# Vandermode/TFPnP

Measured on AMD Instinct MI355X. Metric: PnP-ADMM iters/sec (and images/sec) at env_batch=48, 256x256, 30 inner iters, higher is better.
Workload: dtype f32 (v_mfma_f32_32x32x2_f32; Winograd F(2x2,3x3) on the layers with cout % 32 == 0); 1 GPU; CS-MRI ADMM 256x256 env_batch=48/GPU radial x4 sigma_n=15, 6 solver calls x 5 inner iters + PSNR reward, no early stop; global_batch=48, parallelism=single GPU

## Files before the change

### include/pnpx.h

```cpp
#ifndef PNPX_H
#define PNPX_H

#include <stddef.h>
#include <stdint.h>

#ifdef __cplusplus
extern "C" {
#endif

typedef struct pnpx_ctx pnpx_ctx;

enum pnpx_status {
  PNPX_OK = 0,
  PNPX_ERR_ARG = 1,
  PNPX_ERR_SHAPE = 2,
  PNPX_ERR_NO_WEIGHTS = 3,
  PNPX_ERR_ALLOC = 4,
  PNPX_ERR_HIP = 5,
  PNPX_ERR_RANGE = 6
};

const char* pnpx_version(void);
const char* pnpx_last_error(void);

// ... 167 lines not shown
int pnpx_spi_admm_train(pnpx_ctx* ctx, const float* vars_in, float* vars_out, const float* x0, const float* Kmap,
                        const float* sigma_d, const float* mu, int param_stride, int B, int H, int W, int T,
                        float* saved, unsigned long long* ticket, void* stream);
int pnpx_spi_admm_backward(pnpx_ctx* ctx, const float* x0, const float* Kmap, const float* sigma_d, const float* mu,
                           int param_stride, const float* saved, const float* grad_vars_out, float* grad_vars_in,
                           float* grad_sigma_d, float* grad_mu, float* work, int B, int H, int W, int T,
                           unsigned long long ticket, void* stream);

int pnpx_radon_det_count(int R);
int pnpx_radon_forward(pnpx_ctx* ctx, const float* img, float* sino, int B, int R, int n_view, void* stream);
int pnpx_radon_backprojection(pnpx_ctx* ctx, const float* sino, float* img, int B, int R, int n_view,
                              void* stream);
int pnpx_ct_iadmm(pnpx_ctx* ctx, const float* vars_in, float* vars_out, const float* y0, int n_view,
                  float opnorm, const float* sigma_d, const float* mu, const float* tau, int param_stride,
                  int B, int R, int T, void* stream);
int pnpx_ct_iadmm_train(pnpx_ctx* ctx, const float* vars_in, float* vars_out, const float* y0, int n_view,
                        float opnorm, const float* sigma_d, const float* mu, const float* tau, int param_stride, int B,
                        int R, int T, float* saved, unsigned long long* ticket, void* stream);
int pnpx_ct_iadmm_backward(pnpx_ctx* ctx, int n_view, float opnorm, const float* sigma_d, const float* mu,
                           const float* tau, int param_stride, const float* saved, const float* grad_vars_out,
                           float* grad_vars_in, float* grad_sigma_d, float* grad_mu, float* grad_tau, float* work,
                           int B, int R, int T, unsigned long long ticket, void* stream);
int pnpx_ct_pg(pnpx_ctx* ctx, const float* vars_in, float* vars_out, const float* y0, int n_view,
               float opnorm, const float* sigma_d, const float* tau, int param_stride, int B, int R, int T,
               void* stream);
int pnpx_ct_pg_train(pnpx_ctx* ctx, const float* vars_in, float* vars_out, const float* y0, int n_view, float opnorm,
                     const float* sigma_d, const float* tau, int param_stride, int B, int R, int T, float* saved,
                     unsigned long long* ticket, void* stream);
int pnpx_ct_pg_backward(pnpx_ctx* ctx, int n_view, float opnorm, const float* sigma_d, const float* tau,
                        int param_stride, const float* saved, const float* grad_vars_out, float* grad_vars_in,
                        float* grad_sigma_d, float* grad_tau, float* work, int B, int R, int T,
                        unsigned long long ticket, void* stream);

#ifdef __cplusplus
}
#endif
#endif
```

### tfpnp_amd/_lib.py

```python
import ctypes as C
import os
import threading

import torch

_HERE = os.path.dirname(os.path.abspath(__file__))
LIB_PATH = os.environ.get("PNPX_LIB", os.path.join(_HERE, "libpnpx.so"))

_lib = None
_lock = threading.Lock()

c_float_p = C.POINTER(C.c_float)
c_void_p = C.c_void_p


class PnpxError(RuntimeError):
    pass


PNPX_ERR_RANGE = 6


_P = c_void_p
_SIGNATURES = {
# ... 78 lines not shown
    "pnpx_csmri_redadmm_train": (C.c_int, [c_void_p, _P, _P, _P, _P, _P, _P, _P] + [C.c_int] * 5 +
                                 [_P, C.POINTER(C.c_ulonglong), c_void_p]),
    "pnpx_csmri_redadmm_backward": (C.c_int, [c_void_p, _P, _P, _P, _P, _P, C.c_int, _P, _P, _P, _P, _P, _P, _P] +
                                    [C.c_int] * 4 + [C.c_ulonglong, c_void_p]),
    "pnpx_csmri_redadmm": (C.c_int, [c_void_p, _P, _P, _P, _P, _P, _P, _P] + [C.c_int] * 5 + [c_void_p]),
    "pnpx_pr_iadmm_train": (C.c_int, [c_void_p, _P, _P, _P, _P, _P, _P, _P] + [C.c_int] * 6 +
                            [_P, C.POINTER(C.c_ulonglong), c_void_p]),
    "pnpx_pr_iadmm_backward": (C.c_int, [c_void_p, _P, _P, _P, _P, _P, C.c_int, _P, _P, _P, _P, _P, _P, _P] + [C.c_int] * 5 +
                               [C.c_ulonglong, c_void_p]),
    "pnpx_pr_iadmm": (C.c_int, [c_void_p, _P, _P, _P, _P, _P, _P, _P] + [C.c_int] * 6 + [c_void_p]),
    "pnpx_pr_pg_train": (C.c_int, [c_void_p, _P, _P, _P, _P, _P, _P] + [C.c_int] * 6 +
                         [_P, C.POINTER(C.c_ulonglong), c_void_p]),
    "pnpx_pr_pg_backward": (C.c_int, [c_void_p, _P, _P, _P, _P, C.c_int, _P, _P, _P, _P, _P, _P] + [C.c_int] * 5 +
                            [C.c_ulonglong, c_void_p]),
    "pnpx_pr_pg": (C.c_int, [c_void_p, _P, _P, _P, _P, _P, _P] + [C.c_int] * 6 + [c_void_p]),
    "pnpx_spi_admm_train": (C.c_int, [c_void_p, _P, _P, _P, _P, _P, _P] + [C.c_int] * 5 +
                            [_P, C.POINTER(C.c_ulonglong), c_void_p]),
    "pnpx_spi_admm_backward": (C.c_int, [c_void_p, _P, _P, _P, _P, C.c_int, _P, _P, _P, _P, _P, _P] + [C.c_int] * 4 +
                               [C.c_ulonglong, c_void_p]),
    "pnpx_spi_admm": (C.c_int, [c_void_p, _P, _P, _P, _P, _P, _P] + [C.c_int] * 5 + [c_void_p]),
    "pnpx_radon_det_count": (C.c_int, [C.c_int]),
    "pnpx_radon_forward": (C.c_int, [c_void_p, _P, _P, C.c_int, C.c_int, C.c_int, c_void_p]),
    "pnpx_radon_backprojection": (C.c_int, [c_void_p, _P, _P, C.c_int, C.c_int, C.c_int, c_void_p]),
    "pnpx_ct_iadmm_train": (C.c_int, [c_void_p, _P, _P, _P, C.c_int, C.c_float, _P, _P, _P] + [C.c_int] * 4 +
                            [_P, C.POINTER(C.c_ulonglong), c_void_p]),
    "pnpx_ct_iadmm_backward": (C.c_int, [c_void_p, C.c_int, C.c_float, _P, _P, _P, C.c_int, _P, _P, _P, _P, _P, _P, _P] +
                               [C.c_int] * 3 + [C.c_ulonglong, c_void_p]),
    "pnpx_ct_pg_train": (C.c_int, [c_void_p, _P, _P, _P, C.c_int, C.c_float, _P, _P] + [C.c_int] * 4 +
                         [_P, C.POINTER(C.c_ulonglong), c_void_p]),
    "pnpx_ct_pg_backward": (C.c_int, [c_void_p, C.c_int, C.c_float, _P, _P, C.c_int, _P, _P, _P, _P, _P, _P] +
                            [C.c_int] * 3 + [C.c_ulonglong, c_void_p]),
    "pnpx_ct_iadmm": (C.c_int, [c_void_p, _P, _P, _P, C.c_int, C.c_float, _P, _P, _P] + [C.c_int] * 4 + [c_void_p]),
    "pnpx_ct_pg": (C.c_int, [c_void_p, _P, _P, _P, C.c_int, C.c_float, _P, _P] + [C.c_int] * 4 + [c_void_p]),
}
EXPORTED_SYMBOLS = tuple(_SIGNATURES)


def lib():
    global _lib
    if _lib is None:
        with _lock:
            if _lib is None:
                if not os.path.exists(LIB_PATH):
                    raise PnpxError(
                        f"{LIB_PATH} not found: the HIP library has not been built "
                        "(run `make -C tfpnp_amd/csrc` or __graft_entry__.build()). There is no CPU fallback.")
                l = C.CDLL(LIB_PATH)
                missing = []
                for name, (res, args) in _SIGNATURES.items():
                    try:
                        fn = getattr(l, name)
                    except AttributeError:
                        if "PNPX_LIB" in os.environ:
                            missing.append(name)
                            continue
                        raise
                    fn.restype = res
                    fn.argtypes = args
                if missing:
                    import warnings
                    warnings.warn(f"PNPX_LIB={LIB_PATH} lacks {len(missing)} symbol(s) of include/pnpx.h: "
                                  + ", ".join(missing) + " -- calls to them will fail with AttributeError")
                _lib = l
    return _lib


# ... 5 lines not shown
```

### tfpnp_amd/csrc/api.hip

```cpp
#include <cstring>

#include "common.h"
#include "conv3x3.h"
#include "conv_hs.h"

namespace pnpx {

static thread_local std::string g_err;

void set_error(const char* fmt, ...) {
  char buf[1024];
  va_list ap;
  va_start(ap, fmt);
  vsnprintf(buf, sizeof(buf), fmt, ap);
  va_end(ap);
  g_err = buf;
}

int hip_fail(hipError_t e, const char* what, const char* file, int line) {
  set_error("HIP error %d (%s) at %s:%d in %s", (int)e, hipGetErrorString(e), file, line, what);
  return PNPX_ERR_HIP;
}

int ctx_scratch(pnpx_ctx* ctx, size_t bytes, void** out) {
// ... 322 lines not shown
  if (is("policy_s2_hs") && (value == 0 || value == 1)) return PNPX_OK;
  if (is("fold_first") && (value == 0 || value == 1)) {
    ctx->opt_fold_first = value;
    return PNPX_OK;
  }
  if (is("fft_tile") && value >= 0 && value <= 8192) {
    ctx->opt_fft_tile = value;
    return PNPX_OK;
  }
  if (is("fp32_winograd") && (value == 0 || value == 1)) {
    ctx->opt_fp32_winograd = value;
    return PNPX_OK;
  }
  if (is("fp32_chains") && value >= 0 && value <= 8) {
    ctx->opt_fp32_chains = value;
    return PNPX_OK;
  }
  if (is("fp32_fuse_up") && (value == 0 || value == 1)) {
    ctx->opt_fp32_fuse_up = value;
    return PNPX_OK;
  }
  if (is("fp32_ksplit") && value >= 0 && value <= 2) {
    ctx->opt_fp32_ksplit = value;
    return PNPX_OK;
  }
  if (is("fp32_ksplit_rule") && value >= 1 && value < 256) {
    ctx->opt_ksplit_rule = value;
    return PNPX_OK;
  }
  if (is("fp32_wino8_layers") && value >= 0 && value < (1 << 27)) {
    ctx->opt_fp32_wino8 = value;
    return PNPX_OK;
  }
  if (is("fft_fast") && (value == 0 || value == 1)) {
    ctx->opt_fft_fast = value;
    return PNPX_OK;
  }
  if (is("fft_affine") && (value == 0 || value == 1)) {
    ctx->opt_fft_affine = value;
    return PNPX_OK;
  }
  if (is("chains") && value >= 0 && value <= 8) {
    ctx->opt_chains = value;
    return PNPX_OK;
  }
  if (is("wreg") && value >= 0 && value <= 2) {
    ctx->opt_wreg = value;
    return PNPX_OK;
  }
  if (is("fuse_up") && (value >= 0 && value <= 2)) {
    ctx->opt_fuse_up = value;
    return PNPX_OK;
  }
  if (is("range_guard") && value >= 0 && value <= 2) {
    PNPX_HIP(hipDeviceSynchronize());
    ctx->opt_range_guard = value;
    ctx->range_tripped = false;
    *ctx->range_flag_host = 0;
    return PNPX_OK;
  }
  if (is("train_cache_gb") && value >= -1) {
    ctx->opt_train_cache_gb = value;
    ctx->train_alloc_failed = false;
    ctx->train_budget_bytes = 0;
    if (value == 0) pnpx::train_cache_free(ctx);
    return PNPX_OK;
  }
  if (is("train_cache_release")) {
    pnpx::train_cache_free(ctx);
    ctx->train_alloc_failed = false;
    ctx->train_budget_bytes = 0;
    return PNPX_OK;
  }
  set_error("pnpx_ctx_set_option: unknown option '%s' or bad value %d", key ? key : "(null)", value);
  return PNPX_ERR_ARG;
}

int pnpx_ctx_get_option(pnpx_ctx* ctx, const char* key, int* value) {
  LOCK_CTX(ctx);
  auto is = [&](const char* k) { return key && !std::strcmp(key, k); };
  if (!value) {
    set_error("pnpx_ctx_get_option: null value pointer");
    return PNPX_ERR_ARG;
  }
  if (is("conv_mode")) *value = ctx->conv_mode;
  else if (is("drunet_shift")) *value = ctx->drunet.shift;
  else if (is("subbatch")) *value = ctx->opt_subbatch;
  else if (is("fuse_pool")) *value = ctx->opt_fuse_pool;
  else if (is("fuse_outc")) *value = ctx->opt_fuse_outc;
  else if (is("fuse_first")) *value = ctx->opt_fuse_first;
  else if (is("fuse_up")) *value = ctx->opt_fuse_up;
  else if (is("wreg")) *value = ctx->opt_wreg;
  else if (is("chains")) *value = ctx->opt_chains;
  else if (is("fold_first")) *value = ctx->opt_fold_first;
  else if (is("policy_s2_hs")) *value = 1;
  else if (is("fft_affine")) *value = ctx->opt_fft_affine;
  else if (is("fft_fast")) *value = ctx->opt_fft_fast;
  else if (is("fp32_winograd")) *value = ctx->opt_fp32_winograd;
  else if (is("fp32_wino8_layers")) *value = ctx->opt_fp32_wino8;
  else if (is("fp32_fuse_up")) *value = ctx->opt_fp32_fuse_up;
  else if (is("fp32_ksplit")) *value = ctx->opt_fp32_ksplit;
  else if (is("fp32_ksplit_rule")) *value = ctx->opt_ksplit_rule;
  else if (is("fp32_chains")) *value = ctx->opt_fp32_chains;
  else if (is("fft_tile")) *value = ctx->opt_fft_tile;
  else if (is("range_guard")) *value = ctx->opt_range_guard;
  else if (is("train_cache_gb")) *value = ctx->opt_train_cache_gb;
  else {
    set_error("pnpx_ctx_get_option: unknown option '%s'", key ? key : "(null)");
    return PNPX_ERR_ARG;
  }
  return PNPX_OK;
}

int pnpx_ctx_status(pnpx_ctx* ctx) {
  LOCK_CTX(ctx);
  range_guard_enter(ctx);
  if (ctx->range_tripped) {
    if (ctx->drunet.loaded)
      set_error("half-split range guard tripped: an activation of an earlier DRUNet call left the f16 hi/lo range (|v| >= 4095 "
                "or NaN); that call's output is invalid.  The context now runs %s (the bias-free network is positively "
                "homogeneous: inputs scaled by 2^-%d, the tail multiplies back; a trip at 2^-8 selects exact fp32); acknowledge "
                "with pnpx_ctx_set_option(ctx, \"range_guard\", 1)", ctx->conv_mode == CONV_HS ? "re-scaled passes" : "conv_mode 0",
                ctx->drunet.shift);
    else
    set_error("half-split range guard tripped: an activation of an earlier call left the f16 hi/lo range (|v| >= 4095 or "
              "NaN); that call's output is invalid.  The context now runs conv_mode 0 (exact fp32 MFMA); re-arm with "
              "pnpx_ctx_set_option(ctx, \"range_guard\", 1)");
    return PNPX_ERR_RANGE;
  }
  return PNPX_OK;
}

// ... 69 lines not shown
  }
  size_t hoff[27];
  float hscale[27];
  for (int i = 0; i < 27; ++i) {
    const int mt = conv_hs_mt(L[i].cout);
    const int cin_pad = (L[i].cin + 15) / 16 * 16;
    align();
    hoff[i] = host.size();
    const size_t n16 = (size_t)L[i].cout * cin_pad * 9 * 2;
    host.resize(host.size() + (n16 + 1) / 2, 0.f);
    const float* wsrc = params_host;
    for (int k = 0; k < i; ++k) wsrc += (size_t)L[k].cin * L[k].cout * 9 + L[k].cout;
    hscale[i] = pack_conv_weights_hs(wsrc, L[i].cout, L[i].cin, mt, reinterpret_cast<uint16_t*>(host.data() + hoff[i]));
    ctx->conv_hs[i].cin = L[i].cin;
    ctx->conv_hs[i].cout = L[i].cout;
    ctx->conv_hs[i].cin_pad = cin_pad;
    ctx->conv_hs[i].mt = mt;
    ctx->conv_hs[i].inv_scale = 1.0f / (hscale[i] * HS_ASCALE);
  }
  size_t toff[27];
  for (int i = 0; i < 27; ++i) {
    const int cout_pad = (L[i].cin + 31) / 32 * 32;
    const int mt = (cout_pad % 64 == 0) ? 64 : 32;
    align();
    toff[i] = host.size();
    host.resize(host.size() + (size_t)cout_pad * L[i].cout * 9);
    const float* wsrc = params_host;
    for (int k = 0; k < i; ++k) wsrc += (size_t)L[k].cin * L[k].cout * 9 + L[k].cout;
    pack_conv_weights_transposed(wsrc, L[i].cout, L[i].cin, cout_pad, mt, 8, host.data() + toff[i]);
    ctx->conv_bwd[i].cin = L[i].cout;
    ctx->conv_bwd[i].cout = cout_pad;
    ctx->conv_bwd[i].mt = mt;
    ctx->conv_bwd[i].cc = 8;
  }
  size_t thoff[27], tuoff[27];
  float thscale[27];
  {
    std::vector<float> wt;
    for (int i = 0; i < 27; ++i) {
      const int cin_t = L[i].cout;
      const int cout_t = (L[i].cin + 31) / 32 * 32;
      const int mt = (cout_t % 64 == 0) ? 64 : 32;
      const float* wsrc = params_host;
      for (int k = 0; k < i; ++k) wsrc += (size_t)L[k].cin * L[k].cout * 9 + L[k].cout;
      wt.assign((size_t)cout_t * cin_t * 9, 0.f);
      for (int ci = 0; ci < L[i].cin; ++ci)
        for (int co = 0; co < cin_t; ++co)
          for (int tap = 0; tap < 9; ++tap)
            wt[((size_t)ci * cin_t + co) * 9 + tap] = wsrc[((size_t)co * L[i].cin + ci) * 9 + (8 - tap)];
      align();
      thoff[i] = host.size();
      const size_t n16 = (size_t)cout_t * cin_t * 9 * 2;
      host.resize(host.size() + (n16 + 1) / 2, 0.f);
      thscale[i] = pack_conv_weights_hs(wt.data(), cout_t, cin_t, mt, reinterpret_cast<uint16_t*>(host.data() + thoff[i]));
      tuoff[i] = 0;
      if (conv3x3_wino_packs(cout_t, cin_t)) {
        align();
        tuoff[i] = host.size();
        host.resize(host.size() + conv3x3_wino_floats(cout_t, cin_t));
        pack_conv_weights_wino(wt.data(), cout_t, cin_t, host.data() + tuoff[i]);
      }
      ctx->conv_hs_bwd[i].cin = cin_t;
      ctx->conv_hs_bwd[i].cout = cout_t;
      ctx->conv_hs_bwd[i].cin_pad = cin_t;
      ctx->conv_hs_bwd[i].mt = mt;
      ctx->conv_hs_bwd[i].inv_scale = 1.0f / (thscale[i] * HS_ASCALE);
    }
  }
  align();
  const size_t oc0 = host.size();
  host.insert(host.end(), params_host, params_host + 32 * 2 * 9);
  align();
  const size_t ozero = host.size();
  host.resize(host.size() + 768, 0.f);
  align();
  const size_t ow = host.size();
  host.insert(host.end(), src, src + 32);
  src += 32;
  align();
  const size_t ob = host.size();
  host.push_back(*src);
  host.resize(host.size() + 1024, 0.f);
  PNPX_HIP(hipDeviceSynchronize());
  if (ctx->weights.p) PNPX_HIP(hipFree(ctx->weights.p));
  ctx->weights = DeviceBuf();
  ctx->has_weights = false;
  void* p = nullptr;
  hipError_t e = hipMalloc(&p, host.size() * sizeof(float));
  if (e != hipSuccess) {
    set_error("weight allocation of %zu bytes failed: %s", host.size() * sizeof(float), hipGetErrorString(e));
    return PNPX_ERR_ALLOC;
  }
  PNPX_HIP(hipMemcpy(p, host.data(), host.size() * sizeof(float), hipMemcpyHostToDevice));
  float* d = static_cast<float*>(p);
  for (int i = 0; i < 27; ++i) {
    ctx->conv[i].w = d + woff[i];
    ctx->conv[i].b = d + boff[i];
    ctx->conv_wino_u[i] = uoff[i] ? d + uoff[i] : nullptr;
    ctx->conv_wino_u_bwd[i] = tuoff[i] ? d + tuoff[i] : nullptr;
    ctx->conv_hs[i].w = reinterpret_cast<char*>(d + hoff[i]);
    ctx->conv_bwd[i].w = d + toff[i];
    ctx->conv_bwd[i].b = nullptr;
    ctx->conv_hs_bwd[i].w = reinterpret_cast<char*>(d + thoff[i]);
  }
  ctx->conv0_w = d + oc0;
  ctx->zero_bias = d + ozero;
  ctx->outc_w = d + ow;
  ctx->outc_b = d + ob;
  ctx->weights.p = p;
  ctx->weights.bytes = host.size() * sizeof(float);
  ctx->has_weights = true;
  pnpx::train_cache_free(ctx);
  return PNPX_OK;
}

int pnpx_unet_denoise(pnpx_ctx* ctx, const float* x, const float* sigma, float* out, float* out_preclamp, int B,
                      int H, int W, void* stream) {
  LOCK_CTX(ctx);
  return pnpx::guarded(ctx, static_cast<hipStream_t>(stream), [&]() -> int {
  if (!x || !sigma || !out) {
    set_error("pnpx_unet_denoise: null pointer");
    return PNPX_ERR_ARG;
  }
  return unet_denoise(ctx, x, sigma, 1, out, out_preclamp, B, H, W, static_cast<hipStream_t>(stream), nullptr);
  });
}

int pnpx_unet_denoise_backward(pnpx_ctx* ctx, const float* x, const float* sigma, const float* grad_out, float* grad_x,
                               float* grad_sigma, int B, int H, int W, void* stream) {
  LOCK_CTX(ctx);
  return pnpx::guarded(ctx, static_cast<hipStream_t>(stream), [&]() -> int {
  if (!x || !sigma || !grad_out || !grad_x || !grad_sigma) {
// ... 75 lines not shown
```

### tfpnp_amd/csrc/common.h

```cpp
#pragma once
#include <hip/hip_runtime.h>

#include <cstdarg>
#include <cstdint>
#include <cstdio>
#include <map>
#include <mutex>
#include <string>
#include <vector>

#include "pnpx.h"

namespace pnpx {

void set_error(const char* fmt, ...);
int hip_fail(hipError_t e, const char* what, const char* file, int line);

#define PNPX_HIP(expr)                                                       \
  do {                                                                       \
    hipError_t _e = (expr);                                                  \
    if (_e != hipSuccess) return ::pnpx::hip_fail(_e, #expr, __FILE__, __LINE__); \
  } while (0)
#define PNPX_TRY(expr)          \
  do {                          \
// ... 130 lines not shown

struct pnpx_ctx {
  int device = 0;
  std::mutex mu;
  bool has_weights = false;
  pnpx::ConvLayer conv[27];
  pnpx::ConvLayerHsDev conv_hs[27];
  int conv_mode = pnpx::CONV_F32;
  int opt_subbatch = 24;
  int opt_fuse_pool = 1;
  int opt_fuse_outc = 1;
  int opt_fuse_first = 1;
  int opt_fuse_up = 1;
  int opt_fold_first = 0;
  int opt_fft_tile = 0;
  int opt_fft_fast = 1;
  int opt_fft_affine = 1;
  int lds_block_limit = 0;
  int opt_chains = 0;
  std::vector<hipStream_t> side_streams;
  std::vector<hipEvent_t> ev_pool;
  size_t ev_next = 0;
  int opt_wreg = 2;
  int opt_range_guard = 1;
  int opt_train_cache_gb = -1;
  size_t train_budget_bytes = 0;
  unsigned* range_flag_host = nullptr;
  unsigned* range_flag_dev = nullptr;
  bool range_tripped = false;
  float* conv_wino_u[27] = {};
  float* conv_wino_u_bwd[27] = {};
  int opt_fp32_winograd = 1;
  int opt_fp32_wino8 = (1 << 27) - 1;
  int opt_fp32_chains = 2;
  int opt_fp32_ksplit = 1;
  int opt_ksplit_rule = 1;
  int opt_fp32_fuse_up = 1;
  pnpx::ConvLayer conv_bwd[27];
  pnpx::ConvLayerHsDev conv_hs_bwd[27];
  float* zero_bias = nullptr;
  float* conv0_w = nullptr;
  float* outc_w = nullptr;
  float* outc_b = nullptr;
  pnpx::DeviceBuf weights;
  pnpx::UNetArena arena, arena_grad;
  struct TrainSlot {
    pnpx::UNetArena arena;
    pnpx::DeviceBuf pre;
    unsigned long long ticket = 0;
    int B = 0;
  };
  std::vector<TrainSlot> train_ring;
  unsigned long long train_counter = 0;
  int train_H = 0, train_W = 0, train_mode = -1;
  bool train_alloc_failed = false;
  pnpx::PolicyNet policy;
  pnpx::CriticNet critic;
  pnpx::DruNet drunet;
  pnpx::DeviceBuf scratch;
  std::map<int, float2*> twiddle;
  std::vector<hipEvent_t> events;
};

namespace pnpx {

int chain_event(pnpx_ctx* ctx, hipEvent_t* ev);
// ... 128 lines not shown
```

### tfpnp_amd/csrc/conv3x3.h

```cpp
#pragma once
#include "common.h"

namespace pnpx {

struct ConvArgs {
  const float* in0;
  const float* in1;
  const float* wpk;
  const float* bias;
  float* out;
  int C0, C1;
  int H, W, Hp, Wp;
  int tilesX, tilesY, nct;
  float slope;
  int mode;
  const float* dmask;
  const char* dmask_hs = nullptr;
  const float* res = nullptr;
};

int conv_pack_mt(int cout);
int conv_pack_cc(int cin);
void pack_conv_weights(const float* w, int cout, int cin, int mt, int cc, float* dst);
int launch_conv3x3(const ConvLayer& L, const float* in0, int C0, const float* in1, int C1, float* out, int B,
                   int H, int W, hipStream_t s);
int launch_conv3x3_act(const ConvLayer& L, const float* in0, int C0, const float* in1, int C1, float* out, int B,
                       int H, int W, float slope, const float* res, hipStream_t s);
int launch_conv1x1_act(const ConvLayer& L, const float* in0, float* out, int B, int H, int W, float slope, const float* res, hipStream_t s);
void pack_conv_weights_1x1(const float* w, int cout, int cin, float* dst);
int launch_conv3x3_grad(const ConvLayer& L, const float* gin, float* gout, const float* dmask, int B, int H, int W,
                        hipStream_t s, const char* dmask_hs = nullptr, float mask_slope = 0.2f);
bool conv3x3_wino_ok(int C0, int C1, int cout, int H, int W);
bool conv3x3_wino_packs(int cout, int cin);
size_t conv3x3_wino_floats(int cout, int cin);
void pack_conv_weights_wino(const float* w, int cout, int cin, float* dst);
int launch_conv3x3_wino(const float* u, const float* bias, int cout, const float* in0, int C0, const float* in1, int C1,
                        float* out, int B, int H, int W, hipStream_t s, float slope = 0.2f, const float* res = nullptr,
                        float* pool_out = nullptr);
bool conv3x3_wino_outc_ok(int cin, int cout, int H, int W);
int launch_conv3x3_wino_outc(const float* u, const float* bias, const float* in0, int cin, const float* outc_w, const float* outc_b,
                             const float* x_img, float* img, float* img_pre, int B, int H, int W, hipStream_t s);
bool conv3x3_wino8_ok(int C0, int C1, int cout, int H, int W);
int launch_conv3x3_wino8(const float* u, const float* bias, int cout, const float* in0, int C0, const float* in1, int C1,
                         float* out, int B, int H, int W, hipStream_t s, float slope = 0.2f, const float* res = nullptr,
                         float* pool_out = nullptr, float* ks_part = nullptr, int ks_rule = 1);
int conv3x3_wino8_ksplit(int C0, int C1, int cout, int H, int W, int rule = 1);
size_t conv3x3_wino8_ksplit_bytes_per_image();
int launch_conv3x3_wino8_grad(const float* u, const float* zero_bias, int cout, const float* gin, int cin, float* gout, const float* dmask,
                              float mask_slope, int B, int H, int W, hipStream_t s);
bool conv3x3_wino8_ups_ok(int C0, int C1, int cout, int H, int W);
int launch_conv3x3_wino8_ups(const float* u, const float* bias, int cout, const float* in0, int C0, const float* in1_lowres, int C1,
                             float* out, int B, int H, int W, hipStream_t s, float slope = 0.2f);
int launch_conv3x3_wino8_outc(const float* u, const float* bias, const float* in0, int cin, const float* outc_w, const float* outc_b,
                              const float* x_img, float* img, float* img_pre, int B, int H, int W, hipStream_t s);
void pack_conv_weights_transposed(const float* w, int cout, int cin, int cout_pad, int mt, int cc, float* dst);

}
```

### tfpnp_amd/csrc/unet.hip

```cpp
#include <cstdlib>

#include "common.h"
#include "conv3x3.h"
#include "conv_hs.h"
#include "conv_first.h"
#include "hs_rec.h"
#include "unet_plan.h"

namespace pnpx {

__global__ void prep_input_kernel(const float* __restrict__ x, const float* __restrict__ sigma, int sigma_stride,
                                  float* __restrict__ dst, int H, int W, int Hp, int Wp) {
  const int b = blockIdx.z;
  const int y = blockIdx.y;
  const int xx = blockIdx.x * blockDim.x + threadIdx.x;
  if (xx >= W) return;
  const float v = x[((size_t)b * H + y) * W + xx];
  float* d = dst + (size_t)b * 2 * Hp * Wp + (size_t)(y + 1) * Wp + xx + PADL;
  d[0] = v;
  d[(size_t)Hp * Wp] = sigma[(size_t)b * sigma_stride];
}

__global__ __launch_bounds__(256) void maxpool2_kernel(const float* __restrict__ src, float* __restrict__ dst,
                                                       size_t n_out, int H, int W) {
// ... 504 lines not shown
  }
  if (no_outc_fuse) {
    hipLaunchKernelGGL(outc_residual_hs_kernel, g1d(npix), dim3(256), 0, s, rat(P.y[0], 0), x, ctx->outc_w, ctx->outc_b,
                       out, out_pre, H, W, npix);
    PNPX_LAUNCH_CHECK();
    PNPX_TRY(rec.mark("outc_residual_clamp", 2.0 * 32 * (double)H * W * B));
  }
  return PNPX_OK;
}

static int unet_forward_f32(pnpx_ctx* ctx, UNetArena& ar, const UNetPlan& P, const float* x, const float* sigma, int sigma_stride, float* out,
                            float* out_pre, int B, int H, int W, hipStream_t s, Recorder& rec, bool keep_all, bool level_chains, int b_base = 0, int B_call = 0) {
  if (B_call <= 0) B_call = B;
  char* A = static_cast<char*>(ar.buf.p);
  auto fptr = [&](const Act& d) { return reinterpret_cast<float*>(A + d.off + (size_t)b_base * act_bytes_per_image(CONV_F32, d.C, d.H, d.W)); };
  float* const ks_part0 = reinterpret_cast<float*>(A + P.ks_part + (size_t)b_base * P.ks_part_per_image);
  auto ks_on = [&](int cout, int h, int w) {
    if (ctx->opt_fp32_ksplit == 2) return true;
    return ctx->opt_fp32_ksplit == 1 && (long long)(h / 16) * (w / 16) * (cout / 64) * B_call < 256;
  };
  const bool first_valu = ctx->opt_fuse_first && W % 4 == 0 && ctx->conv[0].cout == 32;
  if (!first_valu) {
    hipLaunchKernelGGL(prep_input_kernel, dim3((W + 63) / 64, H, B), dim3(64), 0, s, x, sigma, sigma_stride, fptr(P.in0), H,
                       W, padded_h(H), padded_w(W));
    PNPX_LAUNCH_CHECK();
    PNPX_TRY(rec.mark("prep_input", 0));
  }
  auto conv = [&](int li, const Act& i0, const Act* i1, const Act& o, const Act* pooled = nullptr, bool* pooled_done = nullptr) -> int {
    const ConvLayer& L = ctx->conv[li];
    const int C1 = i1 ? i1->C : 0;
    if (pooled_done) *pooled_done = false;
    if (ctx->opt_fp32_winograd && ctx->conv_wino_u[li] && conv3x3_wino_ok(i0.C, C1, L.cout, o.H, o.W)) {
      const bool w8 = ((ctx->opt_fp32_wino8 >> li) & 1) && conv3x3_wino8_ok(i0.C, C1, L.cout, o.H, o.W);
      if (w8) {
        const bool ks = ks_on(L.cout, o.H, o.W);
        PNPX_TRY(launch_conv3x3_wino8(ctx->conv_wino_u[li], L.b, L.cout, fptr(i0), i0.C, i1 ? fptr(*i1) : nullptr, C1, fptr(o), B, o.H, o.W, s, 0.2f,
                                      nullptr, pooled ? fptr(*pooled) : nullptr, ks ? ks_part0 : nullptr, ctx->opt_ksplit_rule));
      }
      else
        PNPX_TRY(launch_conv3x3_wino(ctx->conv_wino_u[li], L.b, L.cout, fptr(i0), i0.C, i1 ? fptr(*i1) : nullptr, C1, fptr(o), B, o.H, o.W, s, 0.2f,
                                     nullptr, pooled ? fptr(*pooled) : nullptr));
      if (pooled_done) *pooled_done = pooled != nullptr;
      return rec.mark("conv3x3_wino", 2.0 * 9.0 * L.cin * L.cout * (double)o.H * o.W * B);
    } else {
      PNPX_TRY(launch_conv3x3(L, fptr(i0), i0.C, i1 ? fptr(*i1) : nullptr, C1, fptr(o), B, o.H, o.W, s));
    }
    return rec.mark("conv3x3", 2.0 * 9.0 * L.cin * L.cout * (double)o.H * o.W * B);
  };
  auto block = [&](int li, const Act& i0, const Act* i1, int lvl, const Act& o, const Act* pooled = nullptr, bool* pooled_done = nullptr) -> int {
    const Act& ta = i1 ? P.da[lvl] : P.a[lvl];
    const Act& tb = i1 ? P.db[lvl] : P.b[lvl];
    if (li == 0 && first_valu) {
      hipLaunchKernelGGL(conv_first_f32_kernel, dim3((H * (W / 4) + 255) / 256, 4, B), dim3(256), 0, s, x, sigma, sigma_stride, ctx->conv0_w,
                         ctx->conv[0].b, fptr(ta), H, W, 0.2f);
      PNPX_LAUNCH_CHECK();
      PNPX_TRY(rec.mark("conv3x3", 2.0 * 9.0 * 2 * 32 * (double)H * W * B));
    } else
    PNPX_TRY(conv(li, i0, i1, ta));
    PNPX_TRY(conv(li + 1, ta, nullptr, tb));
    return conv(li + 2, tb, nullptr, o, pooled, pooled_done);
  };
  bool pooled = false;
  PNPX_TRY(block(0, P.in0, nullptr, 0, P.x[0], &P.p[1], &pooled));
  for (int l = 1; l < 5; ++l) {
    const Act& src = P.x[l - 1];
    if (!pooled) {
      const size_t n_pool = (size_t)B * src.C * (src.H / 2) * (src.W / 2);
// ... 167 lines not shown
```

Measured before the change: 114.5 iters/s.

## Add Winograd F(4x4,3x3) fp32 MFMA conv kernel for plain UNet layers

```diff
diff --git a/include/pnpx.h b/include/pnpx.h
--- a/include/pnpx.h
+++ b/include/pnpx.h
@@ -223,6 +223,9 @@
                         float* grad_sigma_d, float* grad_tau, float* work, int B, int R, int T,
                         unsigned long long ticket, void* stream);
 
+void pnpx_winof4_matrices(double* g18, double* bt36, double* at24);
+int pnpx_winof4_pack(const float* w, int cout, int cin, float* dst);
+
 #ifdef __cplusplus
 }
 #endif
diff --git a/tfpnp_amd/_lib.py b/tfpnp_amd/_lib.py
--- a/tfpnp_amd/_lib.py
+++ b/tfpnp_amd/_lib.py
@@ -134,6 +134,8 @@
                             [C.c_int] * 3 + [C.c_ulonglong, c_void_p]),
     "pnpx_ct_iadmm": (C.c_int, [c_void_p, _P, _P, _P, C.c_int, C.c_float, _P, _P, _P] + [C.c_int] * 4 + [c_void_p]),
     "pnpx_ct_pg": (C.c_int, [c_void_p, _P, _P, _P, C.c_int, C.c_float, _P, _P] + [C.c_int] * 4 + [c_void_p]),
+    "pnpx_winof4_matrices": (None, [c_void_p, c_void_p, c_void_p]),
+    "pnpx_winof4_pack": (C.c_int, [c_void_p, C.c_int, C.c_int, c_void_p]),
 }
 EXPORTED_SYMBOLS = tuple(_SIGNATURES)
 
diff --git a/tfpnp_amd/csrc/api.hip b/tfpnp_amd/csrc/api.hip
--- a/tfpnp_amd/csrc/api.hip
+++ b/tfpnp_amd/csrc/api.hip
@@ -378,6 +378,10 @@
     ctx->opt_fp32_wino8 = value;
     return PNPX_OK;
   }
+  if (is("fp32_winof4_layers") && value >= 0 && value < (1 << 27)) {
+    ctx->opt_fp32_winof4 = value;
+    return PNPX_OK;
+  }
   if (is("fft_fast") && (value == 0 || value == 1)) {
     ctx->opt_fft_fast = value;
     return PNPX_OK;
@@ -444,6 +448,7 @@
   else if (is("fft_fast")) *value = ctx->opt_fft_fast;
   else if (is("fp32_winograd")) *value = ctx->opt_fp32_winograd;
   else if (is("fp32_wino8_layers")) *value = ctx->opt_fp32_wino8;
+  else if (is("fp32_winof4_layers")) *value = ctx->opt_fp32_winof4;
   else if (is("fp32_fuse_up")) *value = ctx->opt_fp32_fuse_up;
   else if (is("fp32_ksplit")) *value = ctx->opt_fp32_ksplit;
   else if (is("fp32_ksplit_rule")) *value = ctx->opt_ksplit_rule;
@@ -579,6 +584,21 @@
     ctx->conv_bwd[i].cout = cout_pad;
     ctx->conv_bwd[i].mt = mt;
     ctx->conv_bwd[i].cc = 8;
+  }
+  size_t u4off[27];
+  {
+    const float* wsrc = params_host;
+    for (int i = 0; i < 27; ++i) {
+      u4off[i] = 0;
+      const bool plain = (i >= 3 && i <= 11) || i == 16 || i == 17 || i == 19 || i == 20 || i == 22 || i == 23;
+      if (plain && conv3x3_winof4_ok(L[i].cin, 0, L[i].cout, 16, 32)) {
+        align();
+        u4off[i] = host.size();
+        host.resize(host.size() + conv3x3_winof4_floats(L[i].cout, L[i].cin));
+        pack_conv_weights_winof4(wsrc, L[i].cout, L[i].cin, host.data() + u4off[i]);
+      }
+      wsrc += (size_t)L[i].cin * L[i].cout * 9 + L[i].cout;
+    }
   }
   size_t thoff[27], tuoff[27];
   float thscale[27];
@@ -645,6 +665,7 @@
     ctx->conv[i].b = d + boff[i];
     ctx->conv_wino_u[i] = uoff[i] ? d + uoff[i] : nullptr;
     ctx->conv_wino_u_bwd[i] = tuoff[i] ? d + tuoff[i] : nullptr;
+    ctx->conv_winof4_u[i] = u4off[i] ? d + u4off[i] : nullptr;
     ctx->conv_hs[i].w = reinterpret_cast<char*>(d + hoff[i]);
     ctx->conv_bwd[i].w = d + toff[i];
     ctx->conv_bwd[i].b = nullptr;
diff --git a/tfpnp_amd/csrc/common.h b/tfpnp_amd/csrc/common.h
--- a/tfpnp_amd/csrc/common.h
+++ b/tfpnp_amd/csrc/common.h
@@ -186,6 +186,8 @@
   float* conv_wino_u_bwd[27] = {};
   int opt_fp32_winograd = 1;
   int opt_fp32_wino8 = (1 << 27) - 1;
+  float* conv_winof4_u[27] = {};
+  int opt_fp32_winof4 = (0x1ff << 3) | (3 << 16) | (3 << 19) | (3 << 22);
   int opt_fp32_chains = 2;
   int opt_fp32_ksplit = 1;
   int opt_ksplit_rule = 1;
diff --git a/tfpnp_amd/csrc/conv3x3.h b/tfpnp_amd/csrc/conv3x3.h
--- a/tfpnp_amd/csrc/conv3x3.h
+++ b/tfpnp_amd/csrc/conv3x3.h
@@ -53,6 +53,11 @@
                              float* out, int B, int H, int W, hipStream_t s, float slope = 0.2f);
 int launch_conv3x3_wino8_outc(const float* u, const float* bias, const float* in0, int cin, const float* outc_w, const float* outc_b,
                               const float* x_img, float* img, float* img_pre, int B, int H, int W, hipStream_t s);
+bool conv3x3_winof4_ok(int C0, int C1, int cout, int H, int W);
+size_t conv3x3_winof4_floats(int cout, int cin);
+void pack_conv_weights_winof4(const float* w, int cout, int cin, float* dst);
+int launch_conv3x3_winof4(const float* u, const float* bias, int cout, const float* in0, int C0, float* out, int B, int H, int W, hipStream_t s,
+                          float slope = 0.2f, float* pool_out = nullptr);
 void pack_conv_weights_transposed(const float* w, int cout, int cin, int cout_pad, int mt, int cc, float* dst);
 
 }
diff --git a/tfpnp_amd/csrc/conv3x3_winof4.hip b/tfpnp_amd/csrc/conv3x3_winof4.hip
--- /dev/null
+++ b/tfpnp_amd/csrc/conv3x3_winof4.hip
@@ -0,0 +1,385 @@
+#include <cmath>
+#include <mutex>
+#include <utility>
+#include <vector>
+
+#include "common.h"
+#include "conv3x3.h"
+#include "wino_common.h"
+#include "winof4_mats.h"
+
+namespace pnpx {
+
+namespace {
+
+using namespace wino;
+
+struct CfgF4 {
+  static constexpr int CT = 64, CK = 8;
+  static constexpr int RWL = 40;
+  static constexpr int RPXL = 18 * RWL + 2;
+  static constexpr int RAW_ELEMS = CK * RPXL;
+  static constexpr int RAW_INSTR = (RAW_ELEMS + 63) / 64;
+  static constexpr int RAW_BYTES = RAW_INSTR * 256;
+  static constexpr int RAW_PER_WAVE = (RAW_INSTR + 7) / 8;
+  static constexpr int NRAW = RAW_INSTR / 8;
+  static constexpr int USTG = 2 * 6 * CK * CT * 4;
+  static constexpr int NUW = USTG / 8192;
+  static constexpr int VSTG = 2 * 6 * CK * 32 * 4;
+  static constexpr int OFF_U = 0, OFF_V = 3 * USTG, OFF_RAW = OFF_V + 3 * VSTG;
+  static constexpr int LDS_USED = OFF_RAW + 2 * RAW_BYTES;
+};
+constexpr int LDS_REQF4 = 160 * 1024;
+#ifndef WINOF4_ABL
+#define WINOF4_ABL 0
+#endif
+static_assert(CfgF4::LDS_USED <= LDS_REQF4, "LDS budget");
+
+template <int A>
+__device__ __forceinline__ float bt_row(float d0, float d1, float d2, float d3, float d4, float d5) {
+  if (A == 0) return fmaf(0.25f, d0, fmaf(-1.25f, d2, d4));
+  if (A == 1) return fmaf(-0.25f, d2, d4) + fmaf(-0.25f, d1, d3);
+  if (A == 2) return fmaf(-0.25f, d2, d4) - fmaf(-0.25f, d1, d3);
+  if (A == 3) return fmaf(0.5f, d3 - d1, d4 - d2);
+  if (A == 4) return fmaf(-0.5f, d3 - d1, d4 - d2);
+  return fmaf(0.25f, d1, fmaf(-1.25f, d3, d5));
+}
+__device__ __forceinline__ void at_rows(float m0, float m1, float m2, float m3, float m4, float m5, float& o0, float& o1, float& o2, float& o3) {
+  const float p12 = m1 + m2, m12 = m1 - m2, p34 = m3 + m4, m34 = m3 - m4;
+  o0 = (m0 + p12) + p34;
+  o1 = fmaf(0.5f, m34, m12);
+  o2 = fmaf(0.25f, p34, p12);
+  o3 = fmaf(0.125f, m34, m12) + m5;
+}
+
+__global__ __launch_bounds__(512, 1) void conv3x3_winof4_f32_kernel(WinoArgs a) {
+  using C = CfgF4;
+  constexpr int CK = C::CK, RWL = C::RWL, RPXL = C::RPXL, RAW_BYTES = C::RAW_BYTES, RAW_PER_WAVE = C::RAW_PER_WAVE;
+  constexpr int USTG = C::USTG, NUW = C::NUW, VSTG = C::VSTG, OFF_U = C::OFF_U, OFF_V = C::OFF_V, OFF_RAW = C::OFF_RAW;
+  constexpr int UQ = USTG / 4;
+  extern __shared__ __attribute__((aligned(16))) char lds[];
+  const int tid = threadIdx.x, lane = tid & 63;
+  const int wave = __builtin_amdgcn_readfirstlane(tid >> 6);
+  const int sw = wave & 3;
+  const int HpWp = a.Hp * a.Wp;
+  const unsigned lds0 = (unsigned)(size_t)(lptr_t)lds;
+  const int nregions = a.rx * a.ry * a.B;
+  const int nx = (gridDim.x % 8 == 0 && nregions >= 32) ? 8 : 1;
+  const int xcd = blockIdx.x % nx, slot = blockIdx.x / nx, nslot = gridDim.x / nx;
+
+  struct Tile {
+    const float* s0;
+    const float* w;
+    int ct, b, x0, y0, ok, pad_;
+  };
+  auto decode = [&](int k) {
+    Tile T;
+    const int j = slot + nslot * k;
+    const int q = j / a.nct;
+    T.ct = j - q * a.nct;
+    const int reg = nx * q + xcd;
+    T.ok = reg < nregions;
+    T.pad_ = 0;
+    const int t1 = reg / a.rx;
+    const int tx = reg - t1 * a.rx;
+    const int t2 = t1 / a.ry;
+    const int ty = t1 - t2 * a.ry;
+    T.b = t2;
+    T.x0 = tx * 32;
+    T.y0 = ty * 16;
+    T.s0 = a.in0 + (size_t)T.b * a.C0 * HpWp + (size_t)T.y0 * a.Wp + T.x0 + (PADL - 1);
+    T.w = a.u + (size_t)T.ct * a.nch * 3 * UQ;
+    return T;
+  };
+  auto raw_of = [&](const Tile& X, int c) { return X.s0 + (size_t)CK * c * HpWp; };
+
+  auto sync_all = [&]() {
+    asm volatile("s_waitcnt vmcnt(0) lgkmcnt(0)" ::: "memory");
+    __builtin_amdgcn_s_barrier();
+  };
+
+  unsigned roff[RAW_PER_WAVE];
+#pragma unroll
+  for (int k = 0; k < RAW_PER_WAVE; ++k) {
+    const int idx = (wave + 8 * k) * 64 + lane;
+    const int c = idx / RPXL, r = idx - c * RPXL;
+    const int hy = r / RWL, hx = r - hy * RWL;
+    roff[k] = (c < CK && hy < 18 && hx < 34) ? 4u * (unsigned)(c * HpWp + hy * a.Wp + hx) : 0u;
+  }
+  const unsigned uoff = lane * 16u;
+  auto dma_u_piece = [&](const float* src, int uslot, int k) {
+    if (WINOF4_ABL & 4) return;
+    glds16(src + wave * 256 + k * 2048, uoff, lds0 + OFF_U + uslot * USTG + (wave + 8 * k) * 1024);
+  };
+  auto dma_raw_piece = [&](const float* src, int rbuf, int k) {
+    if (WINOF4_ABL & 2) return;
+    if (k < C::NRAW || wave + 8 * k < C::RAW_INSTR) glds4(src, roff[k], lds0 + OFF_RAW + rbuf * RAW_BYTES + (wave + 8 * k) * 256);
+  };
+  auto dma_u = [&](const float* src, int uslot) {
+#pragma unroll
+    for (int k = 0; k < NUW; ++k) dma_u_piece(src, uslot, k);
+  };
+  auto dma_raw = [&](const float* src, int rbuf) {
+#pragma unroll
+    for (int k = 0; k < RAW_PER_WAVE; ++k) dma_raw_piece(src, rbuf, k);
+  };
+
+  auto body = [&](auto role_tag) {
+  constexpr int P = decltype(role_tag)::value;
+
+  const int t_ks = lane & 1, t_t16 = (lane >> 1) & 15, t_kq = (lane >> 5) | ((sw & 1) << 1), t_wn = sw >> 1;
+  const int t_tile = t_wn * 16 + t_t16;
+  const int t_rd = ((2 * t_kq + t_ks) * RPXL + 4 * (t_tile >> 3) * RWL + 4 * (t_tile & 7)) * 4;
+  const int t_wr = (P * 3 * 2 + t_wn) * 1024 + (t_kq * 16 + t_t16) * 16 + t_ks * 8;
+  auto transform = [&](auto a_tag, int rbuf, int vslot) {
+    constexpr int A = decltype(a_tag)::value;
+    const char* rb = lds + OFF_RAW + rbuf * RAW_BYTES + t_rd;
+    float d[6][6];
+#pragma unroll
+    for (int y = 0; y < 6; ++y) {
+      const bool need = (A == 0) ? (y % 2 == 0) : (A == 5) ? (y % 2 == 1) : (y >= 1 && y <= 4);
+#pragma unroll
+      for (int x = 0; x < 6; x += 2) {
+        if (need) {
+          const f32x2 v = *reinterpret_cast<const f32x2*>(rb + (y * RWL + x) * 4);
+          d[y][x] = v[0];
+          d[y][x + 1] = v[1];
+        } else {
+          d[y][x] = d[y][x + 1] = 0.f;
+        }
+      }
+    }
+    float t[6];
+#pragma unroll
+    for (int x = 0; x < 6; ++x) t[x] = bt_row<A>(d[0][x], d[1][x], d[2][x], d[3][x], d[4][x], d[5][x]);
+    char* vb = lds + OFF_V + vslot * VSTG + t_wr;
+    *reinterpret_cast<f32x2*>(vb) = (f32x2){bt_row<0>(t[0], t[1], t[2], t[3], t[4], t[5]), bt_row<1>(t[0], t[1], t[2], t[3], t[4], t[5])};
+    *reinterpret_cast<f32x2*>(vb + 2048) = (f32x2){bt_row<2>(t[0], t[1], t[2], t[3], t[4], t[5]), bt_row<3>(t[0], t[1], t[2], t[3], t[4], t[5])};
+    *reinterpret_cast<f32x2*>(vb + 4096) = (f32x2){bt_row<4>(t[0], t[1], t[2], t[3], t[4], t[5]), bt_row<5>(t[0], t[1], t[2], t[3], t[4], t[5])};
+  };
+  auto transform_row = [&](auto s_tag, int rbuf) {
+    constexpr int S = decltype(s_tag)::value;
+    if (WINOF4_ABL & 1) return;
+    transform(std::integral_constant<int, 2 * S + P>{}, rbuf, S);
+  };
+
+  const int mb = 2 * (sw & 1) + P, wn = sw >> 1;
+  const int a_lane = mb * 1024 + lane * 16;
+  const int b_lane = wn * 1024 + lane * 16;
+  f32x4 acc[6][6];
+
+  auto stage = [&](auto s_tag, auto wait_tag, const float* u_src, const float* raw_src, int raw_buf, int t_rbuf) {
+    constexpr int S = decltype(s_tag)::value, SN = (S + 1) % 3;
+    constexpr int WAITN = decltype(wait_tag)::value;
+    auto side = [&]() { transform_row(std::integral_constant<int, SN>{}, t_rbuf); };
+    auto piece = [&](int m) {
+      if (m < NUW) dma_u_piece(u_src, (S + 2) % 3, m);
+      if (S == 2 && m >= 4 && m < 4 + RAW_PER_WAVE) dma_raw_piece(raw_src, raw_buf, m - 4);
+    };
+    auto mfmas = [&]() {
+      if (WINOF4_ABL & 16) return;
+      f32x4 af[6], bf[6];
+#pragma unroll
+      for (int q = 0; q < 6; ++q) {
+        af[q] = *reinterpret_cast<const f32x4*>(lds + OFF_U + S * USTG + q * 4096 + a_lane);
+        bf[q] = *reinterpret_cast<const f32x4*>(lds + OFF_V + S * VSTG + q * 2048 + b_lane);
+      }
+      static_for<6>([&](auto q_tag) {
+        constexpr int Q = decltype(q_tag)::value, R = Q / 3, CP = Q % 3;
+#pragma unroll
+        for (int ks = 0; ks < 2; ++ks)
+#pragma unroll
+          for (int pos = 0; pos < 2; ++pos)
+          {
+            acc[2 * S + R][2 * CP + pos] = __builtin_amdgcn_mfma_f32_16x16x4f32(af[Q][2 * ks + pos], bf[Q][2 * ks + pos], acc[2 * S + R][2 * CP + pos], 0, 0, 0);
+            if (!(WINOF4_ABL & 16)) {
+              piece(4 * Q + 2 * ks + pos);
+              __builtin_amdgcn_sched_barrier(0);
+            }
+          }
+      });
+    };
+    if (P == 0) {
+      mfmas();
+      __builtin_amdgcn_sched_barrier(0);
+      side();
+    } else {
+      side();
+      __builtin_amdgcn_sched_barrier(0);
+      mfmas();
+    }
+    asm volatile("s_waitcnt vmcnt(%0) lgkmcnt(0)" ::"n"(WAITN) : "memory");
+    __builtin_amdgcn_s_barrier();
+  };
+
+  auto epilogue = [&](const Tile& T) {
+    const int tile = wn * 16 + (lane & 15), ty = tile >> 3, tx = tile & 7;
+    const int cbase = T.ct * 64 + mb * 16 + 4 * (lane >> 4);
+    float* ob = a.out + ((size_t)T.b * a.Cout + cbase) * HpWp + (size_t)(T.y0 + 4 * ty + 1) * a.Wp + T.x0 + 4 * tx + PADL;
+    const int Hp_pool = padded_h(a.H / 2), Wp_pool = padded_w(a.W / 2);
+    const size_t HpWp_pool = (size_t)Hp_pool * Wp_pool;
+    float* pb = a.pool ? a.pool + ((size_t)T.b * a.Cout + cbase) * HpWp_pool + (size_t)(T.y0 / 2 + 2 * ty + 1) * Wp_pool + T.x0 / 2 + 2 * tx + PADL : nullptr;
+    float bias4[4];
+#pragma unroll
+    for (int j = 0; j < 4; ++j) bias4[j] = a.bias[cbase + j];
+    static_for<4>([&](auto j_tag) {
+      constexpr int j = decltype(j_tag)::value;
+      float s[4][6];
+#pragma unroll
+      for (int b = 0; b < 6; ++b) at_rows(acc[0][b][j], acc[1][b][j], acc[2][b][j], acc[3][b][j], acc[4][b][j], acc[5][b][j], s[0][b], s[1][b], s[2][b], s[3][b]);
+      const float bias = bias4[j];
+      float* o = ob + (size_t)j * HpWp;
+      f32x4 y[4];
+#pragma unroll
+      for (int i = 0; i < 4; ++i) {
+        float y0, y1, y2, y3;
+        at_rows(s[i][0], s[i][1], s[i][2], s[i][3], s[i][4], s[i][5], y0, y1, y2, y3);
+        y0 += bias;
+        y1 += bias;
+        y2 += bias;
+        y3 += bias;
+        y[i] = (f32x4){fmaxf(y0, y0 * a.slope), fmaxf(y1, y1 * a.slope), fmaxf(y2, y2 * a.slope), fmaxf(y3, y3 * a.slope)};
+        if (!(WINOF4_ABL & 32) || a.slope == 123.f) *reinterpret_cast<f32x4*>(o + i * a.Wp) = y[i];
+      }
+      if (a.pool && (!(WINOF4_ABL & 32) || a.slope == 123.f)) {
+        float* p = pb + (size_t)j * HpWp_pool;
+        *reinterpret_cast<f32x2*>(p) = (f32x2){fmaxf(fmaxf(y[0][0], y[0][1]), fmaxf(y[1][0], y[1][1])), fmaxf(fmaxf(y[0][2], y[0][3]), fmaxf(y[1][2], y[1][3]))};
+        *reinterpret_cast<f32x2*>(p + Wp_pool) = (f32x2){fmaxf(fmaxf(y[2][0], y[2][1]), fmaxf(y[3][0], y[3][1])), fmaxf(fmaxf(y[2][2], y[2][3]), fmaxf(y[3][2], y[3][3]))};
+      }
+    });
+  };
+
+  using I0 = std::integral_constant<int, 0>;
+  using I1 = std::integral_constant<int, 1>;
+  using I2 = std::integral_constant<int, 2>;
+  using WaitHalo = std::integral_constant<int, NUW + C::NRAW>;
+  using WaitU = std::integral_constant<int, NUW>;
+
+  int k = 0;
+  Tile T = decode(0);
+  if (!T.ok) return;
+  dma_raw(T.s0, 0);
+  dma_u(T.w, 0);
+  dma_u(T.w + UQ, 1);
+  dma_raw(raw_of(T, 1), 1);
+  sync_all();
+  transform_row(I0{}, 0);
+  sync_all();
+
+  int cc = 0;
+  for (;;) {
+    Tile Tn = decode(k + 1);
+    const bool more = Tn.ok;
+    if (!more) Tn = T;
+#pragma unroll
+    for (int i = 0; i < 6; ++i)
+#pragma unroll
+      for (int j = 0; j < 6; ++j) acc[i][j] = (f32x4){0.f, 0.f, 0.f, 0.f};
+    for (int c = 0; c < a.nch; ++c, ++cc) {
+      const float* w_c = T.w + (size_t)c * 3 * UQ;
+      const float* nu = (c + 1 < a.nch) ? w_c + 3 * UQ : Tn.w;
+      const float* nraw = (c + 2 < a.nch) ? raw_of(T, c + 2) : raw_of(Tn, c + 2 - a.nch);
+      const int rcur = cc & 1;
+      stage(I0{}, WaitHalo{}, w_c + 2 * UQ, nullptr, 0, rcur);
+      stage(I1{}, WaitU{}, nu, nullptr, 0, rcur);
+      stage(I2{}, WaitHalo{}, nu + UQ, nraw, rcur, rcur ^ 1);
+    }
+    if (!(WINOF4_ABL & 8)) epilogue(T);
+    if (!more) break;
+    T = Tn;
+    ++k;
+  }
+  sync_all();
+  };
+  if (wave < 4) body(std::integral_constant<int, 0>{});
+  else body(std::integral_constant<int, 1>{});
+}
+
+}
+
+bool conv3x3_winof4_ok(int C0, int C1, int cout, int H, int W) {
+  return C1 == 0 && C0 >= 16 && C0 % 8 == 0 && cout > 0 && cout % 64 == 0 && H >= 16 && H % 16 == 0 && W >= 32 && W % 32 == 0;
+}
+size_t conv3x3_winof4_floats(int cout, int cin) { return (size_t)36 * cout * cin; }
+
+void pack_conv_weights_winof4(const float* w, int cout, int cin, float* dst) {
+  const int nch = cin / 8;
+  for (int co = 0; co < cout; ++co)
+    for (int ci = 0; ci < cin; ++ci) {
+      const float* g = w + ((size_t)co * cin + ci) * 9;
+      double gg[6][3], u[6][6];
+      for (int i = 0; i < 6; ++i)
+        for (int x = 0; x < 3; ++x) gg[i][x] = WINOF4_G[i][0] * g[0 * 3 + x] + WINOF4_G[i][1] * g[1 * 3 + x] + WINOF4_G[i][2] * g[2 * 3 + x];
+      for (int i = 0; i < 6; ++i)
+        for (int j = 0; j < 6; ++j) u[i][j] = gg[i][0] * WINOF4_G[j][0] + gg[i][1] * WINOF4_G[j][1] + gg[i][2] * WINOF4_G[j][2];
+      const int ct = co / 64, mb = (co % 64) / 16, m = co % 16, ch = ci / 8, kq = (ci % 8) / 2, ks = ci % 2;
+      for (int i = 0; i < 6; ++i)
+        for (int j = 0; j < 6; ++j) {
+          const size_t idx = (((((((((size_t)ct * nch + ch) * 3 + i / 2) * 2 + i % 2) * 3 + j / 2) * 4 + mb) * 4 + kq) * 16 + m) * 2 + ks) * 2 + j % 2;
+          dst[idx] = (float)u[i][j];
+        }
+    }
+}
+
+int launch_conv3x3_winof4(const float* u, const float* bias, int cout, const float* in0, int C0, float* out, int B, int H, int W, hipStream_t s,
+                          float slope, float* pool_out) {
+  if (!conv3x3_winof4_ok(C0, 0, cout, H, W)) {
+    set_error("conv3x3_winof4: unsupported geometry (%d -> %d channels, %d x %d)", C0, cout, H, W);
+    return PNPX_ERR_SHAPE;
+  }
+  WinoArgs a{};
+  a.in0 = in0;
+  a.in1 = in0;
+  a.u = u;
+  a.bias = bias;
+  a.pool = pool_out;
+  a.out = out;
+  a.B = B;
+  a.H = H;
+  a.W = W;
+  a.Hp = padded_h(H);
+  a.Wp = padded_w(W);
+  a.C0 = C0;
+  a.C1 = 0;
+  a.Cout = cout;
+  a.slope = slope;
+  a.nct = cout / 64;
+  a.nch = C0 / CfgF4::CK;
+  a.nch_all = a.nch;
+  a.ksplit = 1;
+  a.rx = W / 32;
+  a.ry = H / 16;
+  static std::once_flag attr_once[64];
+  int dev = 0;
+  PNPX_HIP(hipGetDevice(&dev));
+  if (dev >= 0 && dev < 64) {
+    hipError_t e = hipSuccess;
+    std::call_once(attr_once[dev], [&] {
+      e = hipFuncSetAttribute(reinterpret_cast<const void*>(&conv3x3_winof4_f32_kernel), hipFuncAttributeMaxDynamicSharedMemorySize, LDS_REQF4);
+    });
+    PNPX_HIP(e);
+  }
+  const long long nreg = (long long)a.rx * a.ry * a.B, ntiles = nreg * a.nct;
+  long long grid = 256;
+  if (grid >= ntiles) grid = ntiles;
+  else if ((grid / 8) % a.nct != 0 && grid >= 8LL * a.nct) grid -= grid % (8 * a.nct);
+  hipLaunchKernelGGL(conv3x3_winof4_f32_kernel, dim3((unsigned)grid), dim3(512), LDS_REQF4, s, a);
+  PNPX_LAUNCH_CHECK();
+  return PNPX_OK;
+}
+
+}
+
+extern "C" void pnpx_winof4_matrices(double* g18, double* bt36, double* at24) {
+  for (int i = 0; i < 6; ++i)
+    for (int j = 0; j < 3; ++j) g18[i * 3 + j] = pnpx::WINOF4_G[i][j];
+  for (int i = 0; i < 6; ++i)
+    for (int j = 0; j < 6; ++j) bt36[i * 6 + j] = pnpx::WINOF4_BT[i][j];
+  for (int i = 0; i < 4; ++i)
+    for (int j = 0; j < 6; ++j) at24[i * 6 + j] = pnpx::WINOF4_AT[i][j];
+}
+extern "C" int pnpx_winof4_pack(const float* w, int cout, int cin, float* dst) {
+  if (!w || !dst || cout <= 0 || cout % 64 != 0 || cin <= 0 || cin % 8 != 0) return PNPX_ERR_SHAPE;
+  pnpx::pack_conv_weights_winof4(w, cout, cin, dst);
+  return PNPX_OK;
+}
diff --git a/tfpnp_amd/csrc/unet.hip b/tfpnp_amd/csrc/unet.hip
--- a/tfpnp_amd/csrc/unet.hip
+++ b/tfpnp_amd/csrc/unet.hip
@@ -560,7 +560,12 @@
     if (pooled_done) *pooled_done = false;
     if (ctx->opt_fp32_winograd && ctx->conv_wino_u[li] && conv3x3_wino_ok(i0.C, C1, L.cout, o.H, o.W)) {
       const bool w8 = ((ctx->opt_fp32_wino8 >> li) & 1) && conv3x3_wino8_ok(i0.C, C1, L.cout, o.H, o.W);
-      if (w8) {
+      const bool f4 = w8 && ((ctx->opt_fp32_winof4 >> li) & 1) && ctx->conv_winof4_u[li] && !i1 &&
+                      conv3x3_winof4_ok(i0.C, 0, L.cout, o.H, o.W) &&
+                      !(ks_on(L.cout, o.H, o.W) && conv3x3_wino8_ksplit(i0.C, 0, L.cout, o.H, o.W, ctx->opt_ksplit_rule) > 1);
+      if (f4) {
+        PNPX_TRY(launch_conv3x3_winof4(ctx->conv_winof4_u[li], L.b, L.cout, fptr(i0), i0.C, fptr(o), B, o.H, o.W, s, 0.2f, pooled ? fptr(*pooled) : nullptr));
+      } else if (w8) {
         const bool ks = ks_on(L.cout, o.H, o.W);
         PNPX_TRY(launch_conv3x3_wino8(ctx->conv_wino_u[li], L.b, L.cout, fptr(i0), i0.C, i1 ? fptr(*i1) : nullptr, C1, fptr(o), B, o.H, o.W, s, 0.2f,
                                       nullptr, pooled ? fptr(*pooled) : nullptr, ks ? ks_part0 : nullptr, ctx->opt_ksplit_rule));
diff --git a/tfpnp_amd/csrc/winof4_mats.h b/tfpnp_amd/csrc/winof4_mats.h
--- /dev/null
+++ b/tfpnp_amd/csrc/winof4_mats.h
@@ -0,0 +1,18 @@
+#pragma once
+
+namespace pnpx {
+
+constexpr double WINOF4_G[6][3] = {{4.0, 0.0, 0.0},
+                                   {2.0 / 3.0, 2.0 / 3.0, 2.0 / 3.0},
+                                   {2.0 / 3.0, -2.0 / 3.0, 2.0 / 3.0},
+                                   {-8.0 / 3.0, -4.0 / 3.0, -2.0 / 3.0},
+                                   {-8.0 / 3.0, 4.0 / 3.0, -2.0 / 3.0},
+                                   {0.0, 0.0, 1.0}};
+constexpr double WINOF4_BT[6][6] = {{0.25, 0.0, -1.25, 0.0, 1.0, 0.0},  {0.0, -0.25, -0.25, 1.0, 1.0, 0.0}, {0.0, 0.25, -0.25, -1.0, 1.0, 0.0},
+                                    {0.0, -0.5, -1.0, 0.5, 1.0, 0.0},   {0.0, 0.5, -1.0, -0.5, 1.0, 0.0},   {0.0, 0.25, 0.0, -1.25, 0.0, 1.0}};
+constexpr double WINOF4_AT[4][6] = {{1.0, 1.0, 1.0, 1.0, 1.0, 0.0},
+                                    {0.0, 1.0, -1.0, 0.5, -0.5, 0.0},
+                                    {0.0, 1.0, 1.0, 0.25, 0.25, 0.0},
+                                    {0.0, 1.0, -1.0, 0.125, -0.125, 1.0}};
+
+}
```

Measured after the change: 129.3 iters/s (median of 6 runs). 1.13x the previous value.
